# urbste/pyTheiaSfM

Measured on AMD Instinct MI355X. Metric: BA residuals/sec (LM-iterations/sec x observations); RANSAC hypotheses/sec alongside, higher is better.
Workload: dtype f64; 1 GPU; synth_ba_v1 C4: 1000 views / 500000 tracks / 3001239 observations, mixed pinhole + double-sphere (8 intrinsics groups), TRIVIAL loss, intrinsics NONE, homogeneous-manifold points, 8 LM iterations per solve, use_inner_iterations = false on the GPU and the CPU leg (the trust-region step of north_star alone; the reference's default = true is measured in "with_inner_iterations"); views=1000, tracks=500000, observations=3001239, reduced_system_n=6000, k3_levels=8, fused_kernel_runs=2102, n_ranks_seen_by_rccl=1, n_ranks_in_process_group=1

## Files before the change

include/theia_hip.h:

```cpp
#ifndef THEIA_HIP_H_
#define THEIA_HIP_H_

#include <stddef.h>
#include <stdint.h>

#ifdef __cplusplus
extern "C" {
#endif

enum {
  THEIA_HIP_OK = 0,
  THEIA_HIP_ERR_INVALID_ARGUMENT = -1,
  THEIA_HIP_ERR_NO_DEVICE = -2,
  THEIA_HIP_ERR_UNSUPPORTED = -3,
  THEIA_HIP_ERR_OUT_OF_MEMORY = -4,
  THEIA_HIP_ERR_INTERNAL = -5
};

int theia_hip_init(int device_ordinal);
int theia_hip_shutdown(void);
int theia_hip_device_count(int* count);
const char* theia_hip_last_error(void);
const char* theia_hip_version(void);

// ... 416 lines not shown
  int32_t pos;
  int32_t p4pfr_static_seeded;
  int64_t dls_calls;
} theia_rng_state;

int theia_hip_rng_seed(theia_rng_state* state, uint32_t seed);
int theia_hip_rng_rand_int(theia_rng_state* state, int32_t lo, int32_t hi, int32_t n, int32_t* out);
int theia_hip_rng_rand_double(theia_rng_state* state, double lo, double hi, int32_t n, double* out);
int theia_hip_rng_rand_gaussian(theia_rng_state* state, double mean, double std_dev, int32_t n, double* out);
int theia_hip_rng_discard(theia_rng_state* state, uint64_t words);

typedef struct theia_ransac_streams {
  int32_t num_streams;
  const int32_t* stream_of_problem;
  theia_rng_state* states;
} theia_ransac_streams;

int theia_hip_ransac_estimate_streams(const theia_ransac_batch* batch, const theia_ransac_params* params,
                                      const theia_ransac_streams* streams, theia_ransac_result* result);

int theia_hip_five_point_relative_pose(int32_t num, const double* corr,
                                       double* essential_matrices,
                                       int32_t* num_solutions);
int theia_hip_pose_from_three_points(int32_t num, const double* corr2d3d,
                                     double* rotations, double* translations,
                                     int32_t* num_solutions);
int theia_hip_sqpnp(int32_t num, const int64_t* offsets, const double* features,
                    const double* world_points, double* quaternions,
                    double* translations, int32_t* num_solutions);

int theia_hip_dls_pnp(int32_t num, const int64_t* offsets, const double* features,
                      const double* world_points, const int64_t* call_index,
                      double* quaternions, double* translations, int32_t* num_solutions);
void theia_hip_dls_macaulay_terms(int64_t first_call, int64_t num_calls, double* out);
int theia_hip_four_point_pose_and_focal_length(int32_t num, const double* corr2d3d, double* projection_matrices,
                                               int32_t* num_solutions);
int theia_hip_four_point_focal_length_radial_distortion_ex(int32_t num, const double* corr2d3d, const double* limits,
                                                           const double* rotation_draws, double* models, int32_t* num_solutions,
                                                           int32_t* num_solver_solutions);
int theia_hip_four_point_focal_length_radial_distortion(int32_t num, const double* corr2d3d, const double* limits,
                                                        const double* rotation_draws, double* models, int32_t* num_solutions);

int theia_hip_guided_knn(int32_t num_groups, const int64_t* q_off, const int32_t* q_idx, const int64_t* c_off,
                         const int32_t* c_idx, int32_t n1, int32_t n2, int32_t dim, const float* desc1, const float* desc2,
                         float* nn_dist, int32_t* nn_index);
int theia_hip_randint_stream(uint32_t seed, int32_t n, int32_t lo, int32_t hi, int32_t* out);
int theia_hip_selftest_wave_primitives(int32_t count, int32_t* mismatches);
int theia_hip_selftest_eig_team(int32_t variant, int32_t n, int32_t count, const double* A, const int32_t* active,
                                double* team_out, double* single_out);
int theia_hip_selftest_svd9_team(int32_t team, int32_t with_v, int32_t count, const double* A, double* team_out,
                                 double* single_out);
int theia_hip_selftest_five_point_pre_team(int32_t count, const double* corr, double* team_out, double* single_out);

void theia_hip_release_scratch(void);

#ifdef __cplusplus
}
#endif
#endif
```

pytheiasfm_amd/_capi.py:

```python
import ctypes as C
import os

import numpy as np

_HERE = os.path.dirname(os.path.abspath(__file__))
LIB_PATH = os.environ.get("THEIA_HIP_LIBRARY") or os.path.join(_HERE, "libtheia_hip.so")

THEIA_MAX_INTRINSICS = 10
THEIA_RANSAC_MODEL_STRIDE = 24
THEIA_HIP_ERR_INVALID_ARGUMENT, THEIA_HIP_ERR_NO_DEVICE, THEIA_HIP_ERR_UNSUPPORTED = -1, -2, -3
THEIA_HIP_ERR_OUT_OF_MEMORY, THEIA_HIP_ERR_INTERNAL = -4, -5

c_double_p = C.POINTER(C.c_double)
c_int32_p = C.POINTER(C.c_int32)
c_int64_p = C.POINTER(C.c_int64)
c_uint8_p = C.POINTER(C.c_uint8)


class TheiaHipError(RuntimeError):
    def __init__(self, code, message):
        super().__init__(f"theia_hip error {code}: {message}")
        self.code = code


# ... 130 lines not shown
class LudSummary(C.Structure):
    _fields_ = [("admm_iterations", C.c_int32), ("converged", C.c_int32), ("r_norm", C.c_double), ("s_norm", C.c_double),
                ("primal_eps", C.c_double), ("dual_eps", C.c_double), ("setup_ms", C.c_double), ("factor_ms", C.c_double),
                ("admm_ms", C.c_double)]


class LigtOptions(C.Structure):
    _fields_ = [("max_power_iterations", C.c_int32), ("reserved", C.c_int32), ("eigensolver_threshold", C.c_double)]


class LigtSummary(C.Structure):
    _fields_ = [("num_views_in_system", C.c_int32), ("tracks_used", C.c_int32), ("tracks_skipped", C.c_int32),
                ("num_constraints", C.c_int32), ("iterations", C.c_int32), ("converged", C.c_int32),
                ("sign_votes", C.c_int32), ("flipped", C.c_int32), ("eigenvalue", C.c_double), ("shift", C.c_double),
                ("setup_ms", C.c_double), ("assemble_ms", C.c_double), ("factor_ms", C.c_double), ("eig_ms", C.c_double)]

    def as_dict(self):
        return {name: getattr(self, name) for name, _ in self._fields_}


MFAS_LDS_MAX_VIEWS = 5632


class TranslationFilterOptions(C.Structure):
    _fields_ = [("num_iterations", C.c_int32), ("reserved", C.c_int32), ("translation_projection_tolerance", C.c_double)]


class TranslationFilterStats(C.Structure):
    _fields_ = [("setup_ms", C.c_double), ("rotate_project_ms", C.c_double), ("order_ms", C.c_double),
                ("weights_ms", C.c_double), ("total_ms", C.c_double), ("source_steps", C.c_int64),
                ("argmax_steps", C.c_int64), ("lds_route", C.c_int32), ("order_threads", C.c_int32)]


class K3Info(C.Structure):
    _fields_ = [("dense", C.c_int32), ("levels", C.c_int32), ("num_symm_tiles", C.c_int32),
                ("num_deferred_targets", C.c_int32), ("num_deferred_partials", C.c_int32), ("split_level", C.c_int32),
                ("num_shared_tiles", C.c_int32), ("flops", C.c_double)]

    def as_dict(self):
        return {name: getattr(self, name) for name, _ in self._fields_}


ALLREDUCE_FN = C.CFUNCTYPE(C.c_int, C.c_void_p, C.c_void_p, C.c_size_t, C.c_int, C.c_void_p)

EXPORTED_SYMBOLS = [
    "theia_hip_init", "theia_hip_shutdown", "theia_hip_device_count", "theia_hip_last_error",
    "theia_hip_version", "theia_ba_options_default", "theia_hip_ba_solve", "theia_hip_ba_views_batch", "theia_hip_ba_two_views_angular_batch", "theia_hip_ba_two_views_batch", "theia_hip_optimize_homography_batch", "theia_hip_optimize_fundamental_matrix_batch", "theia_hip_ba_tracks_batch", "theia_hip_track_statistics", "theia_hip_ba_create",
    "theia_hip_ba_reset_parameters", "theia_hip_estimate_tracks", "theia_hip_ba_set_shard", "theia_hip_ba_snapshot_parameters", "theia_hip_ba_restore_parameters", "theia_hip_ba_set_options", "theia_hip_ba_run", "theia_hip_ba_download",
    "theia_hip_ba_destroy", "theia_hip_ba_covariance", "theia_hip_ba_evaluate", "theia_hip_ba_evaluate_ex", "theia_hip_ba_reduced_system",
    "theia_hip_ba_set_allreduce", "theia_hip_ba_set_inner_global", "theia_hip_ba_plan_info", "theia_hip_rccl_unique_id", "theia_hip_rccl_comm_create",
    "theia_hip_optimize_relative_position_batch", "theia_hip_rccl_comm_destroy", "theia_hip_rccl_comm_count", "theia_hip_ba_set_rccl", "theia_hip_dense_spd_solve", "theia_hip_dense_spd_solve_multi", "theia_hip_tile_sparse_spd_solve", "theia_hip_tile_sparse_spd_solve_sharded", "theia_hip_robust_rotation_averaging", "theia_hip_lud_positions", "theia_hip_ligt_positions", "theia_hip_filter_view_pairs_from_relative_translation", "theia_hip_translation_filter_last_stats", "theia_hip_filter_view_pairs_from_orientation", "theia_ransac_params_default",
    "theia_hip_ransac_estimate_batch", "theia_hip_five_point_relative_pose",
    "theia_hip_pose_from_three_points", "theia_hip_sqpnp", "theia_hip_dls_pnp", "theia_hip_dls_macaulay_terms", "theia_hip_four_point_pose_and_focal_length", "theia_hip_four_point_focal_length_radial_distortion", "theia_hip_four_point_focal_length_radial_distortion_ex", "theia_hip_release_scratch", "theia_hip_guided_knn", "theia_hip_randint_stream", "theia_hip_selftest_wave_primitives",
    "theia_hip_selftest_eig_team", "theia_hip_selftest_svd9_team", "theia_hip_selftest_five_point_pre_team",
    "theia_hip_rng_seed", "theia_hip_rng_rand_int", "theia_hip_rng_rand_double", "theia_hip_rng_rand_gaussian", "theia_hip_rng_discard", "theia_hip_ransac_estimate_streams",
]

_lib = None


def lib():
    global _lib
    if _lib is not None:
        return _lib
    if not os.path.exists(LIB_PATH):
        raise ImportError(
            f"{LIB_PATH} is missing: build it with `python __graft_entry__.py` "
            "(pytheiasfm_amd has no CPU fallback)")
    if os.environ.get("THEIA_HIP_NO_TORCH_PRELOAD", "0") != "1":
        try:
            import torch
        except ImportError:
            pass
    L = C.CDLL(LIB_PATH)
    L.theia_hip_last_error.restype = C.c_char_p
    if os.environ.get("THEIA_HIP_ABORT_TRACE") == "1":
        L.theia_hip_debug_install_abort_trace()
    L.theia_hip_version.restype = C.c_char_p
    L.theia_hip_ba_create.argtypes = [C.POINTER(BaProblem), C.POINTER(BaOptions), C.POINTER(C.c_void_p)]
    L.theia_hip_ba_run.argtypes = [C.c_void_p, C.POINTER(BaSummary)]
    L.theia_hip_ba_download.argtypes = [C.c_void_p, C.POINTER(BaProblem)]
    L.theia_hip_ba_reset_parameters.argtypes = [C.c_void_p, C.POINTER(BaProblem)]
    L.theia_hip_ba_set_options.argtypes = [C.c_void_p, C.POINTER(BaOptions)]
    L.theia_hip_ba_destroy.argtypes = [C.c_void_p]
    L.theia_hip_ba_solve.argtypes = [C.POINTER(BaProblem), C.POINTER(BaOptions), C.POINTER(BaSummary)]
    L.theia_hip_ba_evaluate.argtypes = [C.c_void_p, c_double_p, c_double_p, c_double_p, c_double_p, c_uint8_p]
    L.theia_hip_ba_evaluate_ex.argtypes = [C.c_void_p, c_double_p, c_double_p, c_double_p, c_double_p, c_double_p, c_uint8_p]
    L.theia_hip_ba_reduced_system.argtypes = [C.c_void_p, C.c_double, c_int32_p, c_double_p, c_double_p, C.c_int64]
    L.theia_hip_ba_set_allreduce.argtypes = [C.c_void_p, ALLREDUCE_FN, C.c_void_p]
    L.theia_ba_options_default.argtypes = [C.POINTER(BaOptions)]
    L.theia_hip_dense_spd_solve.argtypes = [C.c_int32, c_double_p, c_double_p, c_double_p]
    L.theia_hip_dense_spd_solve_multi.argtypes = [C.c_int32, c_double_p, C.c_int32, c_double_p, c_double_p]
    L.theia_hip_tile_sparse_spd_solve.argtypes = [C.c_int32, C.c_int32, c_uint8_p, C.c_int32, c_double_p, c_double_p,
                                                  c_double_p, C.POINTER(K3Info), c_int32_p, c_int32_p]
    L.theia_hip_tile_sparse_spd_solve_sharded.argtypes = [C.c_int32, C.c_int32, c_uint8_p, c_uint8_p, c_double_p,
                                                          c_double_p, c_double_p, C.POINTER(K3Info)]
    L.theia_hip_robust_rotation_averaging.argtypes = [C.c_int32, c_double_p, c_uint8_p, C.c_int32, c_int32_p, c_double_p,
                                                      C.POINTER(RotationOptions), C.POINTER(RotationSummary)]
    L.theia_hip_lud_positions.argtypes = [C.c_int32, c_double_p, c_uint8_p, C.c_int32, c_int32_p, c_double_p,
                                          C.POINTER(LudOptions), c_double_p, C.POINTER(LudSummary)]
    L.theia_hip_ligt_positions.argtypes = [C.c_int32, c_double_p, C.c_int32, c_int32_p, c_int32_p, c_double_p, C.c_int32,
                                           c_int32_p, c_double_p, C.POINTER(LigtOptions), c_double_p, c_uint8_p,
                                           c_int32_p, c_double_p, c_int32_p, C.POINTER(LigtSummary)]
    L.theia_hip_filter_view_pairs_from_relative_translation.argtypes = [
        C.c_int32, C.c_int32, c_int32_p, c_double_p, c_double_p, C.POINTER(TranslationFilterOptions), C.POINTER(RngState),
        c_double_p, c_uint8_p, c_double_p, c_int32_p, c_double_p, c_double_p]
    L.theia_hip_translation_filter_last_stats.argtypes = [C.POINTER(TranslationFilterStats)]
    L.theia_hip_filter_view_pairs_from_orientation.argtypes = [C.c_int32, C.c_int32, c_int32_p, c_double_p, c_uint8_p,
                                                               c_double_p, C.c_double, c_uint8_p]
    L.theia_hip_selftest_eig_team.argtypes = [C.c_int32, C.c_int32, C.c_int32, c_double_p, c_int32_p, c_double_p, c_double_p]
    L.theia_hip_selftest_svd9_team.argtypes = [C.c_int32, C.c_int32, C.c_int32, c_double_p, c_double_p, c_double_p]
    L.theia_hip_selftest_five_point_pre_team.argtypes = [C.c_int32, c_double_p, c_double_p, c_double_p]
    _lib = L
    return L


def check(rc):
    if rc != 0:
        raise TheiaHipError(rc, lib().theia_hip_last_error().decode())


def ptr(a, ctype):
    if a is None:
        return C.cast(None, C.POINTER(ctype))
    assert a.flags["C_CONTIGUOUS"]
    return a.ctypes.data_as(C.POINTER(ctype))


class FlatProblem:

    def __init__(self, cam_ext, intrinsics, group_model, cam_group, points, obs_uv, obs_cam, obs_pt,
                 cam_const=None, group_const=None, point_const=None, obs_sqrt_info=None, flags=0):
        self.flags = int(flags)
        f8 = lambda a: np.ascontiguousarray(a, dtype=np.float64)
        i4 = lambda a: np.ascontiguousarray(a, dtype=np.int32)
        u1 = lambda a: None if a is None else np.ascontiguousarray(a, dtype=np.uint8)
        self.cam_ext = f8(cam_ext).reshape(-1, 6)
        self.points = f8(points).reshape(-1, 4)
        intr = f8(intrinsics)
        if intr.ndim == 1:
            intr = intr.reshape(1, -1)
        full = np.zeros((intr.shape[0], THEIA_MAX_INTRINSICS))
        full[:, :intr.shape[1]] = intr
        self.intrinsics = full
        self.group_model = i4(group_model).reshape(-1)
        self.cam_group = i4(cam_group).reshape(-1)
        self.obs_uv = f8(obs_uv).reshape(-1, 2)
        self.obs_cam = i4(obs_cam).reshape(-1)
        self.obs_pt = i4(obs_pt).reshape(-1)
        self.cam_const = u1(cam_const)
        self.group_const = u1(group_const)
        self.point_const = u1(point_const)
        self.obs_sqrt_info = None if obs_sqrt_info is None else f8(obs_sqrt_info).reshape(-1, 2)
        assert self.cam_group.shape[0] == self.cam_ext.shape[0]
        assert self.group_model.shape[0] == self.intrinsics.shape[0]
        assert self.obs_cam.shape[0] == self.obs_uv.shape[0] == self.obs_pt.shape[0]
        self.cam_prior_mask = None
        self.priors = {}
        self.obs_kind = None
        self.point_ref_cam = None; self.point_ref_bearing = None; self.point_inverse_depth = None

    def add_depth_priors(self, obs_index, depth, variance=1.0):
        idx = np.asarray(obs_index, dtype=np.int64).reshape(-1)
        depth = np.broadcast_to(np.asarray(depth, dtype=np.float64), idx.shape)
        var = np.broadcast_to(np.asarray(variance, dtype=np.float64), idx.shape)
# ... 97 lines not shown
```

pytheiasfm_amd/csrc/cholesky_device.h:

```cpp
#pragma once
#include <hip/hip_runtime.h>

namespace thip {
namespace chol {

constexpr int NB = 64;
constexpr int LDP = NB + 1;

typedef double double4_t __attribute__((ext_vector_type(4)));

__device__ __forceinline__ double readlane_d(double v, int l) {
  int lo = __double2loint(v), hi = __double2hiint(v);
  lo = __builtin_amdgcn_readlane(lo, l);
  hi = __builtin_amdgcn_readlane(hi, l);
  return __hiloint2double(hi, lo);
}

template <typename FA, typename FB>
__device__ __forceinline__ void wave_gemm32(FA Aop, FB Bop, double4_t (&acc)[2][2], int lane) {
  const int li = lane & 15, lk = lane >> 4;
#pragma unroll
  for (int ti = 0; ti < 2; ++ti)
#pragma unroll
    for (int tj = 0; tj < 2; ++tj) acc[ti][tj] = (double4_t){0.0, 0.0, 0.0, 0.0};
// ... 132 lines not shown
  }
  __syncthreads();
  PSTAMP(3);
#pragma unroll
  for (int h = 0; h < 2; ++h) {
    const int q0 = 2 * h, q1 = 2 * h + 1;
    double4_t t = (double4_t){0.0, 0.0, 0.0, 0.0};
    t = wave_gemm16([&](int r, int k) { return Ls[16 * q1 + r][16 * q0 + k]; },
                    [&](int k, int cc) { return Zs[16 * q0 + k][16 * q0 + cc]; }, t, i);
#pragma unroll
    for (int reg = 0; reg < 4; ++reg) Ls[16 * q0 + lk + 4 * reg][16 * q1 + li] = t[reg];
  }
  __syncthreads();
#pragma unroll
  for (int h = 0; h < 2; ++h) {
    const int q0 = 2 * h, q1 = 2 * h + 1;
    double4_t t = (double4_t){0.0, 0.0, 0.0, 0.0};
    t = wave_gemm16([&](int r, int k) { return Zs[16 * q1 + r][16 * q1 + k]; },
                    [&](int k, int cc) { return Ls[16 * q0 + k][16 * q1 + cc]; }, t, i);
#pragma unroll
    for (int reg = 0; reg < 4; ++reg) Zs[16 * q1 + lk + 4 * reg][16 * q0 + li] = -t[reg];
  }
  __syncthreads();
  PSTAMP(4);
  {
    double4_t acc[2][2];
    wave_gemm32([&](int r, int k) { return Ls[32 + r][k]; }, [&](int k, int cc) { return Zs[k][cc]; }, acc, i);
#pragma unroll
    for (int ti = 0; ti < 2; ++ti)
#pragma unroll
      for (int tj = 0; tj < 2; ++tj)
#pragma unroll
        for (int reg = 0; reg < 4; ++reg) Ls[16 * ti + lk + 4 * reg][32 + 16 * tj + li] = acc[ti][tj][reg];
    __syncthreads();
    wave_gemm32([&](int r, int k) { return Zs[32 + r][32 + k]; }, [&](int k, int cc) { return Ls[k][32 + cc]; }, acc, i);
#pragma unroll
    for (int ti = 0; ti < 2; ++ti)
#pragma unroll
      for (int tj = 0; tj < 2; ++tj)
#pragma unroll
        for (int reg = 0; reg < 4; ++reg) Zs[32 + 16 * ti + lk + 4 * reg][16 * tj + li] = -acc[ti][tj][reg];
  }
  __syncthreads();
  PSTAMP(5);
#pragma unroll 16
  for (int r = 0; r < NB; ++r) Linv[r * NB + i] = Zs[r][i];
  PSTAMP(6);
#undef PSTAMP
#undef PSUB
#undef PSUB0
}


template <bool STORE_L>
__device__ __forceinline__ void potrf64_wg_core(double* __restrict__ A, int lda, int k0, int nb, double (*Ls)[LDP], double (*Zs)[LDP],
                                                double* rdiag, double* __restrict__ Linv, double* __restrict__ fail_flag) {
  const int tid = threadIdx.x, wv = tid >> 6, i = tid & 63;
  const int li = i & 15, lk = i >> 4;
  {
    const int ic = min(i, nb - 1);
    double v[16];
#pragma unroll
    for (int q = 0; q < 16; ++q) v[q] = A[(size_t)(k0 + min(16 * wv + q, nb - 1)) * lda + k0 + ic];
#pragma unroll
    for (int q = 0; q < 16; ++q) {
      const int r = 16 * wv + q;
      Ls[r][i] = (r < nb && i <= r) ? v[q] : ((r == i) ? 1.0 : 0.0);
      Zs[r][i] = 0.0;
    }
  }
  __syncthreads();
  int bad = 0;
  for (int p = 0; p < 4; ++p) {
    const int c0 = 16 * p;
    if (wv == 0) {
      double r16[16];
#pragma unroll
      for (int j = 0; j < 16; ++j) r16[j] = Ls[i][c0 + j];
      double rs[16];
#pragma unroll
      for (int j = 0; j < 16; ++j) {
        Ls[i][c0 + j] = r16[j];
        __builtin_amdgcn_fence(__ATOMIC_ACQ_REL, "wavefront");
        double d = Ls[c0 + j][c0 + j];
        if (!(d > 0.0)) { bad = 1; d = 1.0; }
        double mk[16];
#pragma unroll
        for (int k = j + 1; k < 16; ++k) mk[k] = Ls[c0 + k][c0 + j];
        double w = __builtin_amdgcn_rcp(d);
        w = __builtin_fma(w, __builtin_fma(-d, w, 1.0), w);
        const double t = -(r16[j] * w);
#pragma unroll
        for (int k = j + 1; k < 16; ++k) r16[k] = __builtin_fma(t, mk[k], r16[k]);
        rs[j] = d;
      }
#pragma unroll
      for (int j = 0; j < 16; ++j) {
        const double d = rs[j];
        double rinv = __builtin_amdgcn_rsq(d);
        rinv = rinv * (1.5 - (0.5 * d) * (rinv * rinv));
        rinv = rinv * (1.5 - (0.5 * d) * (rinv * rinv));
        rs[j] = rinv;
      }
#pragma unroll
      for (int j = 0; j < 16; ++j) {
        if (i == 0) rdiag[c0 + j] = rs[j];
        r16[j] = (i >= c0 + j) ? r16[j] * rs[j] : 0.0;
      }
#pragma unroll
      for (int j = 0; j < 16; ++j) Ls[i][c0 + j] = r16[j];
    }
    __syncthreads();
    {
      int t = 0;
      for (int ti = p + 1; ti < 4; ++ti)
        for (int tj = p + 1; tj <= ti; ++tj, ++t) {
          if ((t & 3) != wv) continue;
          double4_t c;
#pragma unroll
          for (int reg = 0; reg < 4; ++reg) c[reg] = Ls[16 * ti + lk + 4 * reg][16 * tj + li];
          c = wave_gemm16([&](int r, int k) { return -Ls[16 * ti + r][c0 + k]; },
                          [&](int k, int cc) { return Ls[16 * tj + cc][c0 + k]; }, c, i);
#pragma unroll
          for (int reg = 0; reg < 4; ++reg) Ls[16 * ti + lk + 4 * reg][16 * tj + li] = c[reg];
        }
    }
    __syncthreads();
  }
  if (STORE_L && i < nb) {
    double v[16];
#pragma unroll
    for (int q = 0; q < 16; ++q) v[q] = Ls[16 * wv + q][i];
#pragma unroll
    for (int q = 0; q < 16; ++q)
      if (16 * wv + q < nb) A[(size_t)(k0 + 16 * wv + q) * lda + k0 + i] = v[q];
  }
  if (bad && tid == 0 && fail_flag) unsafeAtomicAdd(fail_flag, 1.0);
  if (wv == 0) {
    const int q = i >> 4, c = i & 15;
    double z[16];
#pragma unroll
    for (int r = 0; r < 16; ++r) {
      double s0 = (r == c) ? 1.0 : 0.0, s1 = 0.0;
#pragma unroll
      for (int k = 0; k < r; ++k) {
        const double t = Ls[16 * q + r][16 * q + k] * z[k];
        if (k & 1) s1 -= t; else s0 -= t;
      }
      z[r] = (s0 + s1) * rdiag[16 * q + r];
    }
#pragma unroll
    for (int r = 0; r < 16; ++r) Zs[16 * q + r][16 * q + c] = z[r];
  }
  __syncthreads();
  if (wv < 2) {
    const int q0 = 2 * wv, q1 = 2 * wv + 1;
    double4_t t = (double4_t){0.0, 0.0, 0.0, 0.0};
    t = wave_gemm16([&](int r, int k) { return Ls[16 * q1 + r][16 * q0 + k]; },
                    [&](int k, int cc) { return Zs[16 * q0 + k][16 * q0 + cc]; }, t, i);
#pragma unroll
    for (int reg = 0; reg < 4; ++reg) Ls[16 * q0 + lk + 4 * reg][16 * q1 + li] = t[reg];
  }
  __syncthreads();
  if (wv < 2) {
    const int q0 = 2 * wv, q1 = 2 * wv + 1;
    double4_t t = (double4_t){0.0, 0.0, 0.0, 0.0};
    t = wave_gemm16([&](int r, int k) { return Zs[16 * q1 + r][16 * q1 + k]; },
                    [&](int k, int cc) { return Ls[16 * q0 + k][16 * q1 + cc]; }, t, i);
#pragma unroll
    for (int reg = 0; reg < 4; ++reg) Zs[16 * q1 + lk + 4 * reg][16 * q0 + li] = -t[reg];
  }
  __syncthreads();
  {
    const int ti = wv >> 1, tj = wv & 1;
    double4_t acc = (double4_t){0.0, 0.0, 0.0, 0.0};
#pragma unroll
    for (int kk = 0; kk < 32; kk += 4)
      acc = __builtin_amdgcn_mfma_f64_16x16x4f64(Ls[32 + 16 * ti + li][kk + lk], Zs[kk + lk][16 * tj + li], acc, 0, 0, 0);
    __syncthreads();
#pragma unroll
    for (int reg = 0; reg < 4; ++reg) Ls[16 * ti + lk + 4 * reg][32 + 16 * tj + li] = acc[reg];
    __syncthreads();
    acc = (double4_t){0.0, 0.0, 0.0, 0.0};
#pragma unroll
    for (int kk = 0; kk < 32; kk += 4)
      acc = __builtin_amdgcn_mfma_f64_16x16x4f64(Zs[32 + 16 * ti + li][32 + kk + lk], Ls[kk + lk][32 + 16 * tj + li], acc, 0, 0, 0);
#pragma unroll
    for (int reg = 0; reg < 4; ++reg) Zs[32 + 16 * ti + lk + 4 * reg][16 * tj + li] = -acc[reg];
  }
  __syncthreads();
  if (Linv) {
#pragma unroll
    for (int q = 0; q < 16; ++q) Linv[(16 * wv + q) * NB + i] = Zs[16 * wv + q][i];
  }
}

__device__ __forceinline__ void potrf64_wg(double* __restrict__ A, int lda, int k0, int nb,
                                           double* __restrict__ Linv, double* __restrict__ fail_flag) {
  __shared__ double Ls[NB][LDP];
  __shared__ double Zs[NB][LDP];
  __shared__ double rdiag[NB];
  potrf64_wg_core<true>(A, lda, k0, nb, Ls, Zs, rdiag, Linv, fail_flag);
}

}
}
```

pytheiasfm_amd/csrc/sparse_cholesky.hip:

```cpp
#include "ba_kernels.h"
#include "cholesky_device.h"
#include "device_util.h"

#include <algorithm>
#include <cstdlib>
#include <cstdio>
#include <functional>
#include <map>
#include <memory>
#include <vector>

namespace thip {
namespace {

using namespace chol;


__global__ __launch_bounds__(256) void k_sp_potrf(double* __restrict__ A, int lda, const int* __restrict__ items,
                                                  double* __restrict__ Linv, double* __restrict__ fail_flag) {
  const int* it = items + 3 * blockIdx.x;
  potrf64_wg(A, lda, it[0], it[1], Linv + (size_t)it[2] * NB * NB, fail_flag);
}

__device__ __forceinline__ void load_tile(double (*T)[LDP], const double* __restrict__ A, int lda, int row0, int h,
                                          int col0, int w, int tid) {
  double v[16];
#pragma unroll
  for (int q = 0; q < 16; ++q) {
    const int t = tid + 256 * q, r = t >> 6, c = t & 63;
    v[q] = A[(size_t)(row0 + min(r, h - 1)) * lda + col0 + min(c, w - 1)];
  }
#pragma unroll
  for (int q = 0; q < 16; ++q) {
    const int t = tid + 256 * q, r = t >> 6, c = t & 63;
    T[r][c] = (r < h && c < w) ? v[q] : 0.0;
  }
}

__global__ __launch_bounds__(256) void k_sp_trsm(double* __restrict__ A, int lda, const int* __restrict__ items,
                                                 const double* __restrict__ Linv) {
  __shared__ double P[NB][LDP];
  __shared__ double Z[NB][LDP];
  const int* it = items + 5 * blockIdx.x;
  const int row0 = it[0], h = it[1], k0 = it[2], nb = it[3];
  const int tid = threadIdx.x;
  load_tile(Z, Linv + (size_t)it[4] * NB * NB, NB, 0, NB, 0, NB, tid);
  load_tile(P, A, lda, row0, h, k0, nb, tid);
  __syncthreads();
  const int wv = tid >> 6, lane = tid & 63, li = lane & 15, lk = lane >> 4;
  if (16 * wv >= h) return;
  double4_t acc[4];
#pragma unroll
  for (int q = 0; q < 4; ++q) acc[q] = (double4_t){0.0, 0.0, 0.0, 0.0};
#pragma unroll
  for (int kk = 0; kk < NB; kk += 4) {
    const double a = P[16 * wv + li][kk + lk];
#pragma unroll
    for (int q = 0; q < 4; ++q) acc[q] = __builtin_amdgcn_mfma_f64_16x16x4f64(a, Z[16 * q + li][kk + lk], acc[q], 0, 0, 0);
  }
#pragma unroll
  for (int q = 0; q < 4; ++q)
#pragma unroll
    for (int reg = 0; reg < 4; ++reg) {
      const int r = 16 * wv + lk + 4 * reg, c = 16 * q + li;
      if (r < h && c < nb) A[(size_t)(row0 + r) * lda + k0 + c] = acc[q][reg];
    }
}

__global__ __launch_bounds__(256) void k_sp_potrf_trsm(double* __restrict__ A, int lda, const int* __restrict__ potrf_items, int npotrf,
                                                       const int* __restrict__ trsm_items, double* __restrict__ Linv,
                                                       double* __restrict__ fail_flag) {
  __shared__ double Ls[NB][LDP];
  __shared__ double Zs[NB][LDP];
  __shared__ double rdiag[NB];
  if ((int)blockIdx.x < npotrf) {
    const int* it = potrf_items + 3 * blockIdx.x;
    potrf64_wg_core<false>(A, lda, it[0], it[1], Ls, Zs, rdiag, Linv + (size_t)it[2] * NB * NB, fail_flag);
    return;
  }
  const int* it = trsm_items + 5 * ((blockIdx.x - npotrf) >> 2);
  const int rb = (blockIdx.x - npotrf) & 3;
  const int row0 = it[0], h = it[1], k0 = it[2], nb = it[3];
  if (16 * rb >= h) return;
  const int tid = threadIdx.x;
  double pv[4];
#pragma unroll
  for (int q = 0; q < 4; ++q) {
    const int t = tid + 256 * q, r = 16 * rb + (t >> 6), c = t & 63;
    pv[q] = A[(size_t)(row0 + min(r, h - 1)) * lda + k0 + min(c, nb - 1)];
  }
  potrf64_wg_core<false>(A, lda, k0, nb, Ls, Zs, rdiag, nullptr, nullptr);
  __syncthreads();
#pragma unroll
  for (int q = 0; q < 4; ++q) {
    const int t = tid + 256 * q, r = t >> 6, c = t & 63;
    Ls[r][c] = (16 * rb + r < h && c < nb) ? pv[q] : 0.0;
  }
  __syncthreads();
  const int wv = tid >> 6, lane = tid & 63, li = lane & 15, lk = lane >> 4;
  double4_t acc = (double4_t){0.0, 0.0, 0.0, 0.0};
#pragma unroll
  for (int kk = 0; kk < NB; kk += 4)
    acc = __builtin_amdgcn_mfma_f64_16x16x4f64(Ls[li][kk + lk], Zs[16 * wv + li][kk + lk], acc, 0, 0, 0);
#pragma unroll
  for (int reg = 0; reg < 4; ++reg) {
    const int r = 16 * rb + lk + 4 * reg, c = 16 * wv + li;
    if (r < h && c < nb) A[(size_t)(row0 + r) * lda + k0 + c] = acc[reg];
  }
}

__global__ __launch_bounds__(256) void k_sp_update(double* __restrict__ A, int lda, const int* __restrict__ items,
                                                   const int* __restrict__ srcs) {
  __shared__ double Pr[32][LDP];
  __shared__ double Pc[32][LDP];
  const int* it = items + 7 * (blockIdx.x >> 2);
  const int qr = (blockIdx.x >> 1) & 1, qc = blockIdx.x & 1;
  const int row0 = it[0], h = it[1], col0 = it[2], w = it[3], sbeg = it[4], send = it[5], diag = it[6];
  if ((diag && qc > qr) || 32 * qr >= h || 32 * qc >= w) return;
  const int tid = threadIdx.x, wv = tid >> 6, lane = tid & 63, li = lane & 15, lk = lane >> 4;
  const int tr = wv >> 1, tc = wv & 1;
  const int hr = min(32, h - 32 * qr), wc = min(32, w - 32 * qc);
  double4_t cold, acc = (double4_t){0.0, 0.0, 0.0, 0.0};
#pragma unroll
  for (int reg = 0; reg < 4; ++reg) {
    const int r = 32 * qr + 16 * tr + lk + 4 * reg, c = 32 * qc + 16 * tc + li;
    cold[reg] = A[(size_t)(row0 + min(r, h - 1)) * lda + col0 + min(c, w - 1)];
  }
  double vr[8], vc[8];
  int nb = 0;
  auto fetch = [&](int s) {
    const int k0 = srcs[2 * s];
    nb = srcs[2 * s + 1];
#pragma unroll
    for (int q = 0; q < 8; ++q) {
      const int t = tid + 256 * q, r = t >> 6, c = min(t & 63, nb - 1);
      vr[q] = A[(size_t)(row0 + 32 * qr + min(r, hr - 1)) * lda + k0 + c];
      vc[q] = A[(size_t)(col0 + 32 * qc + min(r, wc - 1)) * lda + k0 + c];
    }
  };
  if (sbeg < send) fetch(sbeg);
  for (int s = sbeg; s < send; ++s) {
    if (s > sbeg) __syncthreads();
#pragma unroll
    for (int q = 0; q < 8; ++q) {
      const int t = tid + 256 * q, r = t >> 6, c = t & 63;
      Pr[r][c] = (r < hr && c < nb) ? vr[q] : 0.0;
      Pc[r][c] = (r < wc && c < nb) ? vc[q] : 0.0;
    }
    if (s + 1 < send) fetch(s + 1);
    __syncthreads();
#pragma unroll
    for (int kk = 0; kk < NB; kk += 4)
      acc = __builtin_amdgcn_mfma_f64_16x16x4f64(Pr[16 * tr + li][kk + lk], Pc[16 * tc + li][kk + lk], acc, 0, 0, 0);
  }
#pragma unroll
  for (int reg = 0; reg < 4; ++reg) {
    const int r = 32 * qr + 16 * tr + lk + 4 * reg, c = 32 * qc + 16 * tc + li;
    if (r < h && c < w && (!diag || c <= r)) A[(size_t)(row0 + r) * lda + col0 + c] = cold[reg] - acc[reg];
  }
}

// ... 12 lines not shown
    const int hr = min(32, h - 32 * qr), wc = min(32, w - 32 * qc);
    double vr[8], vc[8];
    int nb = 0;
    auto fetch = [&](int s) {
      const int k0 = srcs[2 * s];
      nb = srcs[2 * s + 1];
#pragma unroll
      for (int q = 0; q < 8; ++q) {
        const int t = tid + 256 * q, r = t >> 6, c = min(t & 63, nb - 1);
        vr[q] = A[(size_t)(row0 + 32 * qr + min(r, hr - 1)) * lda + k0 + c];
        vc[q] = A[(size_t)(col0 + 32 * qc + min(r, wc - 1)) * lda + k0 + c];
      }
    };
    if (sbeg < send) fetch(sbeg);
    for (int s = sbeg; s < send; ++s) {
      if (s > sbeg) __syncthreads();
#pragma unroll
      for (int q = 0; q < 8; ++q) {
        const int t = tid + 256 * q, r = t >> 6, c = t & 63;
        Pr[r][c] = (r < hr && c < nb) ? vr[q] : 0.0;
        Pc[r][c] = (r < wc && c < nb) ? vc[q] : 0.0;
      }
      if (s + 1 < send) fetch(s + 1);
      __syncthreads();
#pragma unroll
      for (int kk = 0; kk < NB; kk += 4)
        acc = __builtin_amdgcn_mfma_f64_16x16x4f64(Pr[16 * tr + li][kk + lk], Pc[16 * tc + li][kk + lk], acc, 0, 0, 0);
    }
  }
#pragma unroll
  for (int reg = 0; reg < 4; ++reg) out[(32 * qr + 16 * tr + lk + 4 * reg) * NB + 32 * qc + 16 * tc + li] = acc[reg];
}

__global__ __launch_bounds__(256) void k_sp_update_reduce(double* __restrict__ A, int lda, const int* __restrict__ items,
                                                          const double* __restrict__ scratch) {
  const int* it = items + 7 * (blockIdx.x >> 4);
  const int row0 = it[0], h = it[1], col0 = it[2], w = it[3], slot0 = it[4], nslots = it[5], diag = it[6];
  const int e = (blockIdx.x & 15) * 256 + threadIdx.x, r = e >> 6, c = e & 63;
  if (r >= h || c >= w || (diag && c > r)) return;
  const double* src = scratch + (size_t)slot0 * NB * NB + e;
  double v = 0.0;
  int s = 0;
  for (; s + 8 <= nslots; s += 8) {
    double t[8];
#pragma unroll
    for (int u = 0; u < 8; ++u) t[u] = src[(size_t)(s + u) * NB * NB];
#pragma unroll
    for (int u = 0; u < 8; ++u) v += t[u];
  }
  for (; s < nslots; ++s) v += src[(size_t)s * NB * NB];
  A[(size_t)(row0 + r) * lda + col0 + c] -= v;
}

__global__ __launch_bounds__(256) void k_sp_back(const double* __restrict__ A, int lda, const int* __restrict__ items,
                                                 const int* __restrict__ srcs, const double* __restrict__ Linv,
                                                 const double* y, double* x) {
  __shared__ double xs[2][NB], yk[NB], part[4][NB];
  const int* it = items + 5 * blockIdx.x;
  const int k0 = it[0], nb = it[1], sbeg = it[3], send = it[4];
  const double* Z = Linv + (size_t)it[2] * NB * NB;
  const int tid = threadIdx.x, j = tid & 63, ch = tid >> 6;
  double zt[16];
#pragma unroll
  for (int q = 0; q < 16; ++q) zt[q] = Z[(ch * 16 + q) * NB + j];
  const double yv = (tid < nb) ? y[k0 + tid] : 0.0;
  double s = 0.0;
  for (int q = sbeg; q < send; ++q) {
    const int row0 = srcs[2 * q], h = srcs[2 * q + 1];
    const double* col = A + (size_t)row0 * lda + k0 + min(j, nb - 1);
    double v[16];
#pragma unroll
    for (int r = 0; r < 16; ++r) v[r] = col[(size_t)min(ch * 16 + r, h - 1) * lda];
    double* xb = xs[(q - sbeg) & 1];
    if (tid < NB) xb[tid] = (tid < h) ? x[row0 + tid] : 0.0;
    __syncthreads();
#pragma unroll
    for (int r = 0; r < 16; ++r) s += v[r] * xb[ch * 16 + r];
  }
  part[ch][j] = s;
  __syncthreads();
  if (tid < NB) yk[tid] = (tid < nb) ? yv - ((part[0][tid] + part[1][tid]) + (part[2][tid] + part[3][tid])) : 0.0;
  __syncthreads();
  double t = 0.0;
#pragma unroll
  for (int q = 0; q < 16; ++q) { const int r = ch * 16 + q; t += zt[q] * yk[r]; }
  __syncthreads();
  part[ch][j] = t;
  __syncthreads();
  if (tid < nb) x[k0 + tid] = (part[0][tid] + part[1][tid]) + (part[2][tid] + part[3][tid]);
}

__global__ __launch_bounds__(256) void k_sp_symm(double* __restrict__ A, int lda, const int* __restrict__ items) {
  __shared__ double T[NB][LDP];
  const int* it = items + 4 * blockIdx.x;
  const int r0 = it[0], h = it[1], c0 = it[2], w = it[3];
  load_tile(T, A, lda, c0, w, r0, h, threadIdx.x);
  __syncthreads();
#pragma unroll
  for (int q = 0; q < 16; ++q) {
    const int t = threadIdx.x + 256 * q, r = t >> 6, c = t & 63;
    if (r < h && c < w) A[(size_t)(r0 + r) * lda + c0 + c] = T[c][r];
  }
}

struct Level {
  int potrf_off = 0, npotrf = 0, trsm_off = 0, ntrsm = 0, upd_off = 0, nupd = 0, upd_src_off = 0;
  int back_off = 0, nback = 0, back_src_off = 0;
};

struct Orderer {
  const std::vector<std::vector<int>>& nbr;
  std::vector<int> mark, dist, out;
  int stamp = 0;
  explicit Orderer(const std::vector<std::vector<int>>& g) : nbr(g), mark(g.size(), 0), dist(g.size(), 0) {}

  std::vector<int> bfs(int src, int tag) {
    std::vector<int> q{src};
    const int seen = ++stamp;
    std::vector<int>& d = dist;
    d[src] = 0;
    vis.resize(nbr.size());
    vis[src] = seen;
    for (size_t i = 0; i < q.size(); ++i)
      for (int v : nbr[q[i]])
        if (mark[v] == tag && vis[v] != seen) { vis[v] = seen; d[v] = d[q[i]] + 1; q.push_back(v); }
    return q;
  }
  std::vector<int> vis;

  static constexpr int kExact = 8;
// ... 585 lines not shown
  if (!k3_adj_symmetric(nt, tile_adj_union))
    return set_error(THEIA_HIP_ERR_INVALID_ARGUMENT, "tile_sparse_spd_solve_sharded: the tile adjacency is not symmetric");
  for (int t = 0; t < nt; ++t) {
    int c[3] = {0, 0, 0};
    for (int r = 0; r < R; ++r) {
      const uint8_t v = tile_class[(size_t)r * nt + t];
      if (v > 2) return set_error(THEIA_HIP_ERR_INVALID_ARGUMENT, "tile_sparse_spd_solve_sharded: tile class %d", (int)v);
      c[v]++;
    }
    if (!(c[0] == R || (c[1] == 1 && c[2] == R - 1)))
      return set_error(THEIA_HIP_ERR_INVALID_ARGUMENT, "tile_sparse_spd_solve_sharded: tile %d has inconsistent classes across the ranks", t);
  }
  int rc = ensure_device();
  if (rc) return rc;
  std::vector<std::unique_ptr<CholPlan, void (*)(CholPlan*)>> plans;
  for (int r = 0; r < R; ++r) {
    plans.emplace_back(chol_plan_create_sharded(n, tile_adj_union, tile_class + (size_t)r * nt), chol_plan_destroy);
    if (!plans.back()) return set_error(THEIA_HIP_ERR_UNSUPPORTED, "rank %d: no level schedule for this structure", r);
    k3_fill_info(plans.back().get(), info ? info + r : nullptr);
  }
  const std::vector<int>& st = chol_plan_shared_tiles(plans[0].get());
  for (int r = 1; r < R; ++r)
    if (chol_plan_shared_tiles(plans[r].get()) != st) return set_error(THEIA_HIP_ERR_INTERNAL, "rank %d: the shared-tile list differs from rank 0's", r);
  const size_t cnt = (size_t)(n + 1) * n;
  std::vector<DevBuf<double>> dA(R), dw(R);
  DevBuf<double> dsum, dflag;
  if ((rc = dsum.alloc(cnt)) || (rc = dflag.alloc(R))) return rc;
  HIP_TRY(hipMemset(dflag.p, 0, sizeof(double) * R));
  for (int r = 0; r < R; ++r) {
    if ((rc = dA[r].alloc(cnt)) || (rc = dw[r].alloc(dense_cholesky_workspace(n)))) return rc;
    HIP_TRY(hipMemcpy(dA[r].p, A + (size_t)r * n * n, sizeof(double) * (size_t)n * n, hipMemcpyHostToDevice));
    HIP_TRY(hipMemcpy(dA[r].p + (size_t)n * n, b + (size_t)r * n, sizeof(double) * n, hipMemcpyHostToDevice));
    chol_plan_solve_phase(plans[r].get(), 0, dA[r].p, n, dA[r].p + (size_t)n * n, dw[r].p, dflag.p + r, nullptr);
  }
  HIP_TRY(hipGetLastError());
  HIP_TRY(hipDeviceSynchronize());
  std::vector<int> items;
  for (size_t k = 0; k + 1 < st.size(); k += 2) k3_item(items, n, st[k], st[k + 1], 0);
  for (int j = 0; j < nt; ++j) k3_item(items, n, -1, j, 0);
  if ((rc = k3_tiles(dsum.p, dA[0].p, n, items, 0))) return rc;
  for (int r = 1; r < R; ++r) if ((rc = k3_tiles(dsum.p, dA[r].p, n, items, 1))) return rc;
  for (int r = 0; r < R; ++r) if ((rc = k3_tiles(dA[r].p, dsum.p, n, items, 0))) return rc;
  for (int r = 0; r < R; ++r)
    chol_plan_solve_phase(plans[r].get(), 1, dA[r].p, n, dA[r].p + (size_t)n * n, dw[r].p, dflag.p + r, nullptr);
  HIP_TRY(hipGetLastError());
  HIP_TRY(hipDeviceSynchronize());
  std::vector<double> flag(R);
  for (int r = 0; r < R; ++r) HIP_TRY(hipMemcpy(x + (size_t)r * n, dA[r].p + (size_t)n * n, sizeof(double) * n, hipMemcpyDeviceToHost));
  HIP_TRY(hipMemcpy(flag.data(), dflag.p, sizeof(double) * R, hipMemcpyDeviceToHost));
  for (int r = 0; r < R; ++r)
    if (flag[r] != 0.0) return set_error(THEIA_HIP_ERR_INTERNAL, "rank %d: matrix is not positive definite", r);
  return 0;
}
```

Before: 3.704 billion residuals/s.

## Overlap diagonal-block inverse with Cholesky panels and batch back-substitution sources

Restructures the 64x64 workgroup Cholesky so that idle waves compute the triangular inverse of already-factored 16x16 diagonal blocks while other waves still factor later panels. Inverse output goes through an emit callback, which lets the fused potrf+trsm kernel apply the trailing TRSM tiles as each inverse slice becomes ready instead of after the full factorization. The sparse back-substitution now loads four source blocks per barrier instead of one, cutting synchronisation count. Launch bounds request two blocks per CU on the potrf kernels, and a selftest entry point compares the wave and workgroup variants. The risks are extra LDS (a staging Ps tile), register pressure under the new occupancy bound, and subtle inter-wave ordering that now relies on wavefront fences.

```diff
diff --git a/include/theia_hip.h b/include/theia_hip.h
--- a/include/theia_hip.h
+++ b/include/theia_hip.h
@@ -492,6 +492,9 @@
                                  double* single_out);
 int theia_hip_selftest_five_point_pre_team(int32_t count, const double* corr, double* team_out, double* single_out);
 
+int theia_hip_selftest_potrf64(int32_t count, int32_t nb, int32_t lda, int32_t k0, const double* A, double* wave_L,
+                               double* wave_Linv, double* wave_fail, double* wg_L, double* wg_Linv, double* wg_fail);
+
 void theia_hip_release_scratch(void);
 
 #ifdef __cplusplus
diff --git a/pytheiasfm_amd/_capi.py b/pytheiasfm_amd/_capi.py
--- a/pytheiasfm_amd/_capi.py
+++ b/pytheiasfm_amd/_capi.py
@@ -206,7 +206,7 @@
     "theia_hip_optimize_relative_position_batch", "theia_hip_rccl_comm_destroy", "theia_hip_rccl_comm_count", "theia_hip_ba_set_rccl", "theia_hip_dense_spd_solve", "theia_hip_dense_spd_solve_multi", "theia_hip_tile_sparse_spd_solve", "theia_hip_tile_sparse_spd_solve_sharded", "theia_hip_robust_rotation_averaging", "theia_hip_lud_positions", "theia_hip_ligt_positions", "theia_hip_filter_view_pairs_from_relative_translation", "theia_hip_translation_filter_last_stats", "theia_hip_filter_view_pairs_from_orientation", "theia_ransac_params_default",
     "theia_hip_ransac_estimate_batch", "theia_hip_five_point_relative_pose",
     "theia_hip_pose_from_three_points", "theia_hip_sqpnp", "theia_hip_dls_pnp", "theia_hip_dls_macaulay_terms", "theia_hip_four_point_pose_and_focal_length", "theia_hip_four_point_focal_length_radial_distortion", "theia_hip_four_point_focal_length_radial_distortion_ex", "theia_hip_release_scratch", "theia_hip_guided_knn", "theia_hip_randint_stream", "theia_hip_selftest_wave_primitives",
-    "theia_hip_selftest_eig_team", "theia_hip_selftest_svd9_team", "theia_hip_selftest_five_point_pre_team",
+    "theia_hip_selftest_eig_team", "theia_hip_selftest_svd9_team", "theia_hip_selftest_five_point_pre_team", "theia_hip_selftest_potrf64",
     "theia_hip_rng_seed", "theia_hip_rng_rand_int", "theia_hip_rng_rand_double", "theia_hip_rng_rand_gaussian", "theia_hip_rng_discard", "theia_hip_ransac_estimate_streams",
 ]
 
@@ -265,6 +265,7 @@
     L.theia_hip_selftest_eig_team.argtypes = [C.c_int32, C.c_int32, C.c_int32, c_double_p, c_int32_p, c_double_p, c_double_p]
     L.theia_hip_selftest_svd9_team.argtypes = [C.c_int32, C.c_int32, C.c_int32, c_double_p, c_double_p, c_double_p]
     L.theia_hip_selftest_five_point_pre_team.argtypes = [C.c_int32, c_double_p, c_double_p, c_double_p]
+    L.theia_hip_selftest_potrf64.argtypes = [C.c_int32, C.c_int32, C.c_int32, C.c_int32, c_double_p] + [c_double_p] * 6
     _lib = L
     return L
 
diff --git a/pytheiasfm_amd/csrc/cholesky_device.h b/pytheiasfm_amd/csrc/cholesky_device.h
--- a/pytheiasfm_amd/csrc/cholesky_device.h
+++ b/pytheiasfm_amd/csrc/cholesky_device.h
@@ -208,9 +208,9 @@
 }
 
 
-template <bool STORE_L>
-__device__ __forceinline__ void potrf64_wg_core(double* __restrict__ A, int lda, int k0, int nb, double (*Ls)[LDP], double (*Zs)[LDP],
-                                                double* rdiag, double* __restrict__ Linv, double* __restrict__ fail_flag) {
+template <bool STORE_L, typename FStage, typename FEmit>
+__device__ __forceinline__ void potrf64_wg_sched(double* __restrict__ A, int lda, int k0, int nb, double (*Ls)[LDP], double (*Zs)[LDP],
+                                                 double* rdiag, double* __restrict__ fail_flag, FStage stage, FEmit emit) {
   const int tid = threadIdx.x, wv = tid >> 6, i = tid & 63;
   const int li = i & 15, lk = i >> 4;
   {
@@ -225,7 +225,64 @@
       Zs[r][i] = 0.0;
     }
   }
-  __syncthreads();
+  stage();
+  __syncthreads();
+  auto tri_inverse = [&](int q) {
+    const int c = li;
+    double z[16];
+#pragma unroll
+    for (int r = 0; r < 16; ++r) {
+      double s0 = (r == c) ? 1.0 : 0.0, s1 = 0.0;
+#pragma unroll
+      for (int k = 0; k < r; ++k) {
+        const double t = Ls[16 * q + r][16 * q + k] * z[k];
+        if (k & 1) s1 -= t; else s0 -= t;
+      }
+      z[r] = (s0 + s1) * rdiag[16 * q + r];
+    }
+    if (i < 16) {
+#pragma unroll
+      for (int r = 0; r < 16; ++r) Zs[16 * q + r][16 * q + c] = z[r];
+    }
+    __builtin_amdgcn_fence(__ATOMIC_ACQ_REL, "wavefront");
+  };
+  auto t32 = [&](int h) {
+    const int q0 = 2 * h, q1 = 2 * h + 1;
+    double4_t t = (double4_t){0.0, 0.0, 0.0, 0.0};
+    return wave_gemm16([&](int r, int k) { return Ls[16 * q1 + r][16 * q0 + k]; },
+                       [&](int k, int cc) { return Zs[16 * q0 + k][16 * q0 + cc]; }, t, i);
+  };
+  auto z32 = [&](int h, const double4_t& tq) {
+    const int q0 = 2 * h, q1 = 2 * h + 1;
+    double4_t t = (double4_t){0.0, 0.0, 0.0, 0.0};
+#pragma unroll
+    for (int kk = 0; kk < 16; kk += 4)
+      t = __builtin_amdgcn_mfma_f64_16x16x4f64(Zs[16 * q1 + li][16 * q1 + kk + lk], tq[kk >> 2], t, 0, 0, 0);
+#pragma unroll
+    for (int reg = 0; reg < 4; ++reg) Zs[16 * q1 + lk + 4 * reg][16 * q0 + li] = -t[reg];
+    __builtin_amdgcn_fence(__ATOMIC_ACQ_REL, "wavefront");
+  };
+  auto t64 = [&](int tj, double4_t (&t)[2]) {
+#pragma unroll
+    for (int ti = 0; ti < 2; ++ti) {
+      double4_t acc = (double4_t){0.0, 0.0, 0.0, 0.0};
+#pragma unroll
+      for (int kk = 0; kk < 32; kk += 4)
+        acc = __builtin_amdgcn_mfma_f64_16x16x4f64(Ls[32 + 16 * ti + li][kk + lk], Zs[kk + lk][16 * tj + li], acc, 0, 0, 0);
+      t[ti] = acc;
+    }
+  };
+  auto z64 = [&](int ti, int tj, const double4_t (&t)[2]) {
+    double4_t acc = (double4_t){0.0, 0.0, 0.0, 0.0};
+#pragma unroll
+    for (int kk = 0; kk < 32; kk += 4)
+      acc = __builtin_amdgcn_mfma_f64_16x16x4f64(Zs[32 + 16 * ti + li][32 + kk + lk], t[kk >> 4][(kk & 15) >> 2], acc, 0, 0, 0);
+#pragma unroll
+    for (int reg = 0; reg < 4; ++reg) Zs[32 + 16 * ti + lk + 4 * reg][16 * tj + li] = -acc[reg];
+  };
+  double4_t tq = (double4_t){0.0, 0.0, 0.0, 0.0}, ta[2], tb[2];
+#pragma unroll
+  for (int q = 0; q < 2; ++q) ta[q] = tb[q] = (double4_t){0.0, 0.0, 0.0, 0.0};
   int bad = 0;
   for (int p = 0; p < 4; ++p) {
     const int c0 = 16 * p;
@@ -265,8 +322,20 @@
       }
 #pragma unroll
       for (int j = 0; j < 16; ++j) Ls[i][c0 + j] = r16[j];
+    } else if (p > 0) {
+      if (wv == 1) {
+        tri_inverse(p - 1);
+        if (p == 2) z32(0, tq); else tq = t32(p >> 1);
+      } else if (wv == 2) {
+        if (p == 2) emit(0);
+        if (p == 3) { t64(0, ta); t64(1, tb); }
+      } else if (p == 3) {
+        t64(1, tb);
+        emit(1);
+      }
     }
     __syncthreads();
+    if (p == 3) break;
     {
       int t = 0;
       for (int ti = p + 1; ti < 4; ++ti)
@@ -283,72 +352,46 @@
     }
     __syncthreads();
   }
-  if (STORE_L && i < nb) {
+  if (bad && tid == 0 && fail_flag) unsafeAtomicAdd(fail_flag, 1.0);
+  if (wv == 1) {
+    tri_inverse(3);
+    z32(1, tq);
+  } else if (wv == 2) {
+    z64(0, 0, ta);
+    z64(0, 1, tb);
+    __builtin_amdgcn_fence(__ATOMIC_ACQ_REL, "wavefront");
+    emit(2);
+  } else if (STORE_L && i < nb) {
+    const int r0 = wv ? 32 : 0;
+#pragma unroll
+    for (int rb = 0; rb < 32; rb += 16) {
+      double v[16];
+#pragma unroll
+      for (int q = 0; q < 16; ++q) v[q] = Ls[r0 + rb + q][i];
+#pragma unroll
+      for (int q = 0; q < 16; ++q)
+        if (r0 + rb + q < nb) A[(size_t)(k0 + r0 + rb + q) * lda + k0 + i] = v[q];
+    }
+  }
+  __syncthreads();
+  if (wv == 2) z64(1, 0, ta);
+  if (wv == 3) z64(1, 1, tb);
+  __syncthreads();
+  if (wv == 3) emit(3);
+}
+
+template <bool STORE_L>
+__device__ __forceinline__ void potrf64_wg_core(double* __restrict__ A, int lda, int k0, int nb, double (*Ls)[LDP], double (*Zs)[LDP],
+                                                double* rdiag, double* __restrict__ Linv, double* __restrict__ fail_flag) {
+  const int i = threadIdx.x & 63;
+  potrf64_wg_sched<STORE_L>(A, lda, k0, nb, Ls, Zs, rdiag, fail_flag, [] {}, [&](int w) {
+    if (!Linv) return;
     double v[16];
 #pragma unroll
-    for (int q = 0; q < 16; ++q) v[q] = Ls[16 * wv + q][i];
-#pragma unroll
-    for (int q = 0; q < 16; ++q)
-      if (16 * wv + q < nb) A[(size_t)(k0 + 16 * wv + q) * lda + k0 + i] = v[q];
-  }
-  if (bad && tid == 0 && fail_flag) unsafeAtomicAdd(fail_flag, 1.0);
-  if (wv == 0) {
-    const int q = i >> 4, c = i & 15;
-    double z[16];
-#pragma unroll
-    for (int r = 0; r < 16; ++r) {
-      double s0 = (r == c) ? 1.0 : 0.0, s1 = 0.0;
-#pragma unroll
-      for (int k = 0; k < r; ++k) {
-        const double t = Ls[16 * q + r][16 * q + k] * z[k];
-        if (k & 1) s1 -= t; else s0 -= t;
-      }
-      z[r] = (s0 + s1) * rdiag[16 * q + r];
-    }
-#pragma unroll
-    for (int r = 0; r < 16; ++r) Zs[16 * q + r][16 * q + c] = z[r];
-  }
-  __syncthreads();
-  if (wv < 2) {
-    const int q0 = 2 * wv, q1 = 2 * wv + 1;
-    double4_t t = (double4_t){0.0, 0.0, 0.0, 0.0};
-    t = wave_gemm16([&](int r, int k) { return Ls[16 * q1 + r][16 * q0 + k]; },
-                    [&](int k, int cc) { return Zs[16 * q0 + k][16 * q0 + cc]; }, t, i);
-#pragma unroll
-    for (int reg = 0; reg < 4; ++reg) Ls[16 * q0 + lk + 4 * reg][16 * q1 + li] = t[reg];
-  }
-  __syncthreads();
-  if (wv < 2) {
-    const int q0 = 2 * wv, q1 = 2 * wv + 1;
-    double4_t t = (double4_t){0.0, 0.0, 0.0, 0.0};
-    t = wave_gemm16([&](int r, int k) { return Zs[16 * q1 + r][16 * q1 + k]; },
-                    [&](int k, int cc) { return Ls[16 * q0 + k][16 * q1 + cc]; }, t, i);
-#pragma unroll
-    for (int reg = 0; reg < 4; ++reg) Zs[16 * q1 + lk + 4 * reg][16 * q0 + li] = -t[reg];
-  }
-  __syncthreads();
-  {
-    const int ti = wv >> 1, tj = wv & 1;
-    double4_t acc = (double4_t){0.0, 0.0, 0.0, 0.0};
-#pragma unroll
-    for (int kk = 0; kk < 32; kk += 4)
-      acc = __builtin_amdgcn_mfma_f64_16x16x4f64(Ls[32 + 16 * ti + li][kk + lk], Zs[kk + lk][16 * tj + li], acc, 0, 0, 0);
-    __syncthreads();
-#pragma unroll
-    for (int reg = 0; reg < 4; ++reg) Ls[16 * ti + lk + 4 * reg][32 + 16 * tj + li] = acc[reg];
-    __syncthreads();
-    acc = (double4_t){0.0, 0.0, 0.0, 0.0};
-#pragma unroll
-    for (int kk = 0; kk < 32; kk += 4)
-      acc = __builtin_amdgcn_mfma_f64_16x16x4f64(Zs[32 + 16 * ti + li][32 + kk + lk], Ls[kk + lk][32 + 16 * tj + li], acc, 0, 0, 0);
-#pragma unroll
-    for (int reg = 0; reg < 4; ++reg) Zs[32 + 16 * ti + lk + 4 * reg][16 * tj + li] = -acc[reg];
-  }
-  __syncthreads();
-  if (Linv) {
-#pragma unroll
-    for (int q = 0; q < 16; ++q) Linv[(16 * wv + q) * NB + i] = Zs[16 * wv + q][i];
-  }
+    for (int q = 0; q < 16; ++q) v[q] = Zs[16 * w + q][i];
+#pragma unroll
+    for (int q = 0; q < 16; ++q) Linv[(16 * w + q) * NB + i] = v[q];
+  });
 }
 
 __device__ __forceinline__ void potrf64_wg(double* __restrict__ A, int lda, int k0, int nb,
diff --git a/pytheiasfm_amd/csrc/sparse_cholesky.hip b/pytheiasfm_amd/csrc/sparse_cholesky.hip
--- a/pytheiasfm_amd/csrc/sparse_cholesky.hip
+++ b/pytheiasfm_amd/csrc/sparse_cholesky.hip
@@ -16,7 +16,7 @@
 using namespace chol;
 
 
-__global__ __launch_bounds__(256) void k_sp_potrf(double* __restrict__ A, int lda, const int* __restrict__ items,
+__global__ __launch_bounds__(256, 2) void k_sp_potrf(double* __restrict__ A, int lda, const int* __restrict__ items,
                                                   double* __restrict__ Linv, double* __restrict__ fail_flag) {
   const int* it = items + 3 * blockIdx.x;
   potrf64_wg(A, lda, it[0], it[1], Linv + (size_t)it[2] * NB * NB, fail_flag);
@@ -67,12 +67,13 @@
     }
 }
 
-__global__ __launch_bounds__(256) void k_sp_potrf_trsm(double* __restrict__ A, int lda, const int* __restrict__ potrf_items, int npotrf,
+__global__ __launch_bounds__(256, 2) void k_sp_potrf_trsm(double* __restrict__ A, int lda, const int* __restrict__ potrf_items, int npotrf,
                                                        const int* __restrict__ trsm_items, double* __restrict__ Linv,
                                                        double* __restrict__ fail_flag) {
   __shared__ double Ls[NB][LDP];
   __shared__ double Zs[NB][LDP];
   __shared__ double rdiag[NB];
+  __shared__ double Ps[16][LDP];
   if ((int)blockIdx.x < npotrf) {
     const int* it = potrf_items + 3 * blockIdx.x;
     potrf64_wg_core<false>(A, lda, it[0], it[1], Ls, Zs, rdiag, Linv + (size_t)it[2] * NB * NB, fail_flag);
@@ -82,31 +83,32 @@
   const int rb = (blockIdx.x - npotrf) & 3;
   const int row0 = it[0], h = it[1], k0 = it[2], nb = it[3];
   if (16 * rb >= h) return;
-  const int tid = threadIdx.x;
+  const int tid = threadIdx.x, lane = tid & 63, li = lane & 15, lk = lane >> 4;
   double pv[4];
 #pragma unroll
   for (int q = 0; q < 4; ++q) {
     const int t = tid + 256 * q, r = 16 * rb + (t >> 6), c = t & 63;
     pv[q] = A[(size_t)(row0 + min(r, h - 1)) * lda + k0 + min(c, nb - 1)];
   }
-  potrf64_wg_core<false>(A, lda, k0, nb, Ls, Zs, rdiag, nullptr, nullptr);
-  __syncthreads();
-#pragma unroll
-  for (int q = 0; q < 4; ++q) {
-    const int t = tid + 256 * q, r = t >> 6, c = t & 63;
-    Ls[r][c] = (16 * rb + r < h && c < nb) ? pv[q] : 0.0;
-  }
-  __syncthreads();
-  const int wv = tid >> 6, lane = tid & 63, li = lane & 15, lk = lane >> 4;
-  double4_t acc = (double4_t){0.0, 0.0, 0.0, 0.0};
-#pragma unroll
-  for (int kk = 0; kk < NB; kk += 4)
-    acc = __builtin_amdgcn_mfma_f64_16x16x4f64(Ls[li][kk + lk], Zs[16 * wv + li][kk + lk], acc, 0, 0, 0);
-#pragma unroll
-  for (int reg = 0; reg < 4; ++reg) {
-    const int r = 16 * rb + lk + 4 * reg, c = 16 * wv + li;
-    if (r < h && c < nb) A[(size_t)(row0 + r) * lda + k0 + c] = acc[reg];
-  }
+  potrf64_wg_sched<false>(A, lda, k0, nb, Ls, Zs, rdiag, nullptr,
+    [&] {
+#pragma unroll
+      for (int q = 0; q < 4; ++q) {
+        const int t = tid + 256 * q, r = t >> 6, c = t & 63;
+        Ps[r][c] = (16 * rb + r < h && c < nb) ? pv[q] : 0.0;
+      }
+    },
+    [&](int w) {
+      double4_t acc = (double4_t){0.0, 0.0, 0.0, 0.0};
+#pragma unroll
+      for (int kk = 0; kk < NB; kk += 4)
+        acc = __builtin_amdgcn_mfma_f64_16x16x4f64(Ps[li][kk + lk], Zs[16 * w + li][kk + lk], acc, 0, 0, 0);
+#pragma unroll
+      for (int reg = 0; reg < 4; ++reg) {
+        const int r = 16 * rb + lk + 4 * reg, c = 16 * w + li;
+        if (r < h && c < nb) A[(size_t)(row0 + r) * lda + k0 + c] = acc[reg];
+      }
+    });
 }
 
 __global__ __launch_bounds__(256) void k_sp_update(double* __restrict__ A, int lda, const int* __restrict__ items,
@@ -225,10 +227,11 @@
   A[(size_t)(row0 + r) * lda + col0 + c] -= v;
 }
 
+constexpr int kBackGroup = 4;
 __global__ __launch_bounds__(256) void k_sp_back(const double* __restrict__ A, int lda, const int* __restrict__ items,
                                                  const int* __restrict__ srcs, const double* __restrict__ Linv,
                                                  const double* y, double* x) {
-  __shared__ double xs[2][NB], yk[NB], part[4][NB];
+  __shared__ double xs[2][kBackGroup][NB], yk[NB], part[4][NB];
   const int* it = items + 5 * blockIdx.x;
   const int k0 = it[0], nb = it[1], sbeg = it[3], send = it[4];
   const double* Z = Linv + (size_t)it[2] * NB * NB;
@@ -238,17 +241,37 @@
   for (int q = 0; q < 16; ++q) zt[q] = Z[(ch * 16 + q) * NB + j];
   const double yv = (tid < nb) ? y[k0 + tid] : 0.0;
   double s = 0.0;
-  for (int q = sbeg; q < send; ++q) {
-    const int row0 = srcs[2 * q], h = srcs[2 * q + 1];
-    const double* col = A + (size_t)row0 * lda + k0 + min(j, nb - 1);
-    double v[16];
-#pragma unroll
-    for (int r = 0; r < 16; ++r) v[r] = col[(size_t)min(ch * 16 + r, h - 1) * lda];
-    double* xb = xs[(q - sbeg) & 1];
-    if (tid < NB) xb[tid] = (tid < h) ? x[row0 + tid] : 0.0;
+  const double* col0 = A + k0 + min(j, nb - 1);
+  for (int q0 = sbeg, grp = 0; q0 < send; q0 += kBackGroup, ++grp) {
+    const int g = min(kBackGroup, send - q0);
+    int row0[kBackGroup], h[kBackGroup];
+#pragma unroll
+    for (int u = 0; u < kBackGroup; ++u) {
+      const int q = min(q0 + u, send - 1);
+      row0[u] = srcs[2 * q]; h[u] = srcs[2 * q + 1];
+    }
+    double v[kBackGroup][16];
+#pragma unroll
+    for (int u = 0; u < kBackGroup; ++u) {
+      if (u >= g) break;
+      const double* col = col0 + (size_t)row0[u] * lda;
+#pragma unroll
+      for (int r = 0; r < 16; ++r) v[u][r] = col[(size_t)min(ch * 16 + r, h[u] - 1) * lda];
+    }
+    double (*xb)[NB] = xs[grp & 1];
+    {
+      int xr = row0[0], xh = h[0];
+#pragma unroll
+      for (int u = 1; u < kBackGroup; ++u) if (ch == u) { xr = row0[u]; xh = h[u]; }
+      if (ch < g) xb[ch][j] = (j < xh) ? x[xr + j] : 0.0;
+    }
     __syncthreads();
 #pragma unroll
-    for (int r = 0; r < 16; ++r) s += v[r] * xb[ch * 16 + r];
+    for (int u = 0; u < kBackGroup; ++u) {
+      if (u >= g) break;
+#pragma unroll
+      for (int r = 0; r < 16; ++r) s += v[u][r] * xb[u][ch * 16 + r];
+    }
   }
   part[ch][j] = s;
   __syncthreads();
@@ -940,3 +963,45 @@
     if (flag[r] != 0.0) return set_error(THEIA_HIP_ERR_INTERNAL, "rank %d: matrix is not positive definite", r);
   return 0;
 }
+
+namespace thip {
+namespace {
+__global__ __launch_bounds__(64) void k_selftest_potrf_wave(double* __restrict__ A, int lda, int k0, int nb, double* __restrict__ Linv,
+                                                            double* __restrict__ flag) {
+  potrf64_wave(A + (size_t)blockIdx.x * lda * lda, lda, k0, nb, Linv + (size_t)blockIdx.x * NB * NB, flag + blockIdx.x);
+}
+__global__ __launch_bounds__(256, 2) void k_selftest_potrf_wg(double* __restrict__ A, int lda, int k0, int nb, double* __restrict__ Linv,
+                                                           double* __restrict__ flag) {
+  potrf64_wg(A + (size_t)blockIdx.x * lda * lda, lda, k0, nb, Linv + (size_t)blockIdx.x * NB * NB, flag + blockIdx.x);
+}
+}
+}
+
+extern "C" int theia_hip_selftest_potrf64(int32_t count, int32_t nb, int32_t lda, int32_t k0, const double* A, double* wave_L,
+                                          double* wave_Linv, double* wave_fail, double* wg_L, double* wg_Linv, double* wg_fail) {
+  if (count < 1 || count > 4096 || nb < 1 || nb > NB || k0 < 0 || lda < 1 || lda > 4096 || k0 + nb > lda)
+    return set_error(THEIA_HIP_ERR_INVALID_ARGUMENT, "selftest_potrf64: count = %d, nb = %d, lda = %d, k0 = %d", count, nb, lda, k0);
+  if (!A || !wave_L || !wave_Linv || !wave_fail || !wg_L || !wg_Linv || !wg_fail)
+    return set_error(THEIA_HIP_ERR_INVALID_ARGUMENT, "selftest_potrf64: null pointer");
+  int rc = ensure_device();
+  if (rc) return rc;
+  const size_t mats = (size_t)count * lda * lda, invs = (size_t)count * NB * NB;
+  DevBuf<double> d1, d4, z1, z4, f1, f4;
+  if ((rc = d1.up(A, mats)) || (rc = d4.up(A, mats)) || (rc = z1.alloc(invs)) || (rc = z4.alloc(invs)) || (rc = f1.alloc(count)) ||
+      (rc = f4.alloc(count)))
+    return rc;
+  HIP_TRY(hipMemset(f1.p, 0, sizeof(double) * count));
+  HIP_TRY(hipMemset(f4.p, 0, sizeof(double) * count));
+  k_selftest_potrf_wave<<<count, 64>>>(d1.p, lda, k0, nb, z1.p, f1.p);
+  HIP_TRY(hipGetLastError());
+  k_selftest_potrf_wg<<<count, 256>>>(d4.p, lda, k0, nb, z4.p, f4.p);
+  HIP_TRY(hipGetLastError());
+  HIP_TRY(hipDeviceSynchronize());
+  HIP_TRY(hipMemcpy(wave_L, d1.p, sizeof(double) * mats, hipMemcpyDeviceToHost));
+  HIP_TRY(hipMemcpy(wg_L, d4.p, sizeof(double) * mats, hipMemcpyDeviceToHost));
+  HIP_TRY(hipMemcpy(wave_Linv, z1.p, sizeof(double) * invs, hipMemcpyDeviceToHost));
+  HIP_TRY(hipMemcpy(wg_Linv, z4.p, sizeof(double) * invs, hipMemcpyDeviceToHost));
+  HIP_TRY(hipMemcpy(wave_fail, f1.p, sizeof(double) * count, hipMemcpyDeviceToHost));
+  HIP_TRY(hipMemcpy(wg_fail, f4.p, sizeof(double) * count, hipMemcpyDeviceToHost));
+  return 0;
+}
```

Result: no change. 3.716 billion residuals/s, median of 3 (+0.3%).
